# submarine0418/underwater_image_enhancement

Measured on AMD Instinct MI355X. Metric: megapixels/sec enhanced, higher is better.
Workload: dtype f32/f64

## Files before the change

underwater_image_enhancement_amd/csrc/api.hip:

```cpp
#include <cstdarg>
#include <cstdio>
#include <cstring>
#include <type_traits>

#include "common.h"

#include <cstdlib>

namespace uwie {

static thread_local char g_err[512] = "";
static thread_local uwie_ctx *g_ctx = nullptr;
static const Tuning g_default_tuning{};

const Tuning &tune() { return g_ctx ? g_ctx->tune : g_default_tuning; }
uwie_ctx *current_ctx() { return g_ctx; }

void set_error(const char *fmt, ...)
{
    va_list ap;
    va_start(ap, fmt);
    vsnprintf(g_err, sizeof g_err, fmt, ap);
    va_end(ap);
}
// ... 198 lines not shown
        const EntryFuse ef{P.qpart, tune().entry_fuse == 2 ? nullptr : P.gray, P.guess, p->gray_shift};
        UWIE_TRY(launch_cast_classify(ctx, d_in, s, P.kind, nullptr, P.scratch, st, then_airlight && quad_from_cast(p, P) ? &ef : nullptr));
        *kind = P.kind;
    }
    return UWIE_OK;
}

int six_airlight(uwie_ctx *ctx, const uint8_t *d_in, const int32_t *kind, Shape s, const uwie_params *p, const Pipe &P,
                 hipStream_t st, bool after_cast = false)
{
    const bool fused = after_cast && quad_from_cast(p, P);
    return launch_airlight(ctx, d_in, kind, P.gray, s, p->min_size, P.A, nullptr, P.scratch, st,
                           fused && tune().entry_fuse != 2 ? 0 : p->gray_shift, fused ? P.qpart : nullptr);
}

int six_dehaze_tail(uwie_ctx *ctx, const uint8_t *d_in, const int32_t *kind, Shape s, const uwie_params *p, const Pipe &P,
                    uint8_t *d_out_u8, float *d_out_f32, hipStream_t st)
{
    const float eps = 1e-6f;
    const int k = p->strategy;
    int t_is_f32 = 0;
    UWIE_TRY(stage_guided(P, s, p, FuseT0Args{d_in, kind, P.A, (float)p->omega, 1e-6f, 1}, st, &t_is_f32));
    SelectPlan plan;
    const double q[4] = {p->L_low, p->L_high, p->wb_percentile, 100 - p->wb_percentile};
    const RestoreSrc src{d_in, kind, P.A, P.t, t_is_f32};
    bool recompute = false;
    if (tune().select_generic) {
        UWIE_TRY(select_begin<float>(s, q, k == 3 ? 4 : 2, P.scratch, st, &plan));
        UWIE_TRY(launch_restore_planar_hist(d_in, kind, P.A, P.t, s, P.F, plan.ghist, st, false, nullptr, t_is_f32));
        UWIE_TRY(select_run(plan, P.F, 1, s, true, st));
    } else {
        recompute = k != 3 && !tune().restore_store;
        const bool predict = k != 3 || tune().lin_predict3;
        UWIE_TRY(select_lin_begin<float>(s, q, k == 3 ? 4 : 2, P.scratch, st, &plan, predict ? &src : nullptr));
        const bool big = (size_t)s.B * s.npx() >= ((size_t)1 << 24) || tune().rank_sweep >= 2;
        if (recompute && plan.predicted && !t_is_f32 && tune().rank_sweep && big && s.npx() >= 4) {
            UWIE_TRY(launch_restore_rank(src, s, plan, st));
            UWIE_TRY(select_rank_run(plan, s, st, src));
        } else {
            UWIE_TRY(launch_restore_planar_hist(d_in, kind, P.A, P.t, s, recompute ? nullptr : P.F, plan.ghist, st, true,
                                                &plan, t_is_f32));
            UWIE_TRY(select_lin_run(plan, P.F, s, st, recompute ? &src : nullptr));
        }
    }
    if (k == 3) {
        UWIE_TRY(select_lerp_chain(plan, s, eps, P.pct, st));
        return launch_tail_plain(P.F, P.pct, 4, eps, 1, s, 0, 1.0, d_out_u8, d_out_f32, st);
    }
    UWIE_TRY(select_lerp(plan, s, P.pct, st));
    return launch_tail_clahe(ctx, P.F, P.pct, 2, eps, 0, s, p->clip_limit, p->tiles_x, p->tiles_y, k == 1 ? 1 : 0,
                             p->gamma, d_out_u8, d_out_f32, P.scratch, st, recompute ? &src : nullptr);
}

int run_six(uwie_ctx *ctx, const uint8_t *d_in, Shape s, const uwie_params *p, const Pipe &P, uint8_t *d_out_u8,
            float *d_out_f32, hipStream_t st)
{
    const int32_t *kind = nullptr;
    const bool dz = p->strategy >= 1 && p->strategy <= 3;
    UWIE_TRY(six_cast(ctx, d_in, s, p, P, &kind, st, dz));
    if (dz) {
        UWIE_TRY(six_airlight(ctx, d_in, kind, s, p, P, st, true));
        return six_dehaze_tail(ctx, d_in, kind, s, p, P, d_out_u8, d_out_f32, st);
    }
    return launch_code_strategy(ctx, d_in, kind, s, p, d_out_u8, d_out_f32, P.scratch, st);
}

int run_dict_dehaze(uwie_ctx *ctx, const uint8_t *d_in, Shape s, const uwie_params *p, const Pipe &P, uint8_t *d_out_u8,
                    float *d_out_f32, hipStream_t st, double *d_out_f64 = nullptr, bool have_airlight = false)
{
// ... 1759 lines not shown
```

underwater_image_enhancement_amd/csrc/common.h:

```cpp
#pragma once
#include <hip/hip_runtime.h>
#include <stddef.h>
#include <stdint.h>

#include "../../include/uwie.h"

namespace uwie {

void set_error(const char *fmt, ...);
#define UWIE_HIP_CHECK(expr)                                                            \
    do {                                                                                \
        hipError_t _e = (expr);                                                         \
        if (_e != hipSuccess) {                                                         \
            ::uwie::set_error("%s failed: %s (%s:%d)", #expr, hipGetErrorString(_e), __FILE__, __LINE__); \
            return UWIE_E_HIP;                                                          \
        }                                                                               \
    } while (0)
#define UWIE_LAUNCH_CHECK() UWIE_HIP_CHECK(hipGetLastError())
#define UWIE_REQUIRE(cond, msg)                 \
    do {                                        \
        if (!(cond)) {                          \
            ::uwie::set_error("%s", msg);       \
            return UWIE_E_INVALID;              \
        }                                       \
// ... 52 lines not shown
#define UWIE_LAUNCH(kernel, ...) UWIE_LAUNCH_AS(#kernel, kernel, __VA_ARGS__)

}

namespace uwie {
struct Tuning {
    int gf_split = 1;
    int gf_bands = 0;
    int select_generic = 0;
    int restore_store = 0;
    int lin_predict3 = 0;
    int lin_cap = 0;
    int lin_no_predict = 0;
    int q_hist = 1;
    int lin_predict_shift = 0;
    int streams = 1;
    int canny_prepass = 1;
    int gf_fuse = 2;
    int rank_sweep = 1;
    int canny_fault_inject = 0;
    int entry_fuse = 1;
};
const Tuning &tune();
uwie_ctx *current_ctx();
}

struct uwie_ctx {
    int device;
    uwie::Tuning tune;
    bool attr_q_tail = false;
    bool attr_cast_resolve = false;
    int attr_gf_fast = 0;
    int attr_gf_split8 = 0;
    int cus = 0;
    uwie::LabTables *d_lab;
    uwie::CastTables *d_cast;
    uwie::Profiler *prof;
    uint32_t *d_status = nullptr;
    hipStream_t aux[4];
    hipEvent_t fork, join[4];
    bool aux_ready;
    bool last_enhance_f64 = false;
};

namespace uwie {

struct Carver {
    char *base;
    size_t off;
    explicit Carver(void *b) : base(static_cast<char *>(b)), off(0) {}
    template <typename T>
    T *take(size_t count)
    {
        off = (off + 255) & ~size_t(255);
        T *p = base ? reinterpret_cast<T *>(base + off) : nullptr;
        off += count * sizeof(T);
        return p;
    }
    size_t total() const { return (off + 255) & ~size_t(255); }
};

static inline int cdiv(long long a, long long b) { return (int)((a + b - 1) / b); }
static inline int grid_for(size_t n, size_t cap = 8192)
{
    size_t g = (n + 255) / 256;
    if (g > cap) g = cap;
// ... 131 lines not shown
struct FuseT0Args {
    const uint8_t *rgb;
    const int32_t *kind;
    const float *A;
    float omega, norm_eps;
    int pre_clip;
};
int launch_guided_plan(const GuidedPlan &g, Shape s, const uint8_t *d_gray, const void *d_t0, double *d_t, void *ws, hipStream_t st,
                       const FuseT0Args *frame = nullptr);
int guided_fast_th(Shape s, int k);
int launch_guided_fast(const uint8_t *d_gray, const float *d_t0, Shape s, int k, int TH, double eps, double *d_t, hipStream_t st);

constexpr int kMaxPct = 4;
size_t select_ws_bytes(Shape s);
template <typename V>
int launch_percentiles(const V *d_vals, int planar, Shape s, const double *q_percent, int nq, V *d_out, void *ws, hipStream_t st);
int launch_widen_f32(const float *d_in, double *d_out, size_t n, hipStream_t st);

constexpr int kSelGroupStride = 2 * kMaxPct * 2048;
constexpr int kSelOsStride = 2 * kMaxPct;
struct LinState;
struct SelectPlan {
    void *state;
    uint32_t *ghist;
    void *os;
    double t[kMaxPct];
    int nq;
    bool is64;
    LinState *lin;
    void *lists;
    uint32_t *flags;
    uint32_t cap;
    bool predicted;
    uint32_t ranks[2 * kMaxPct];
    template <typename V>
    V *lists_as() const { return static_cast<V *>(lists); }
};
constexpr int kLinBins = 2050;
__host__ __device__ inline uint32_t lin_digit(float x)
{
    if (!(x > 0.0f)) return 0;
    if (x >= 1.0f) return kLinBins - 1;
    const uint32_t d = (uint32_t)(x * 2048.0f);
    return 1 + (d > 2047u ? 2047u : d);
}
__host__ __device__ inline uint32_t lin_digit(double x)
{
    if (!(x > 0.0)) return 0;
    if (x >= 1.0) return kLinBins - 1;
    const uint32_t d = (uint32_t)(x * 2048.0);
    return 1 + (d > 2047u ? 2047u : d);
}
constexpr int kLinLists = 2 * kMaxPct;
constexpr uint32_t kLinNoWin = 0x80000000u;
struct LinState {
    uint32_t rr[2 * kMaxPct];
    uint32_t qbin[2 * kMaxPct];
    uint32_t gid[2 * kMaxPct];
    uint32_t gbin[2 * kMaxPct];
    uint32_t gcount[kLinLists];
    uint32_t ngroups;
    uint32_t wlo[kMaxPct], wspan[kMaxPct];
    uint32_t below[kMaxPct];
};
constexpr int kRankCapMul = 4;
constexpr uint32_t kLinAnyBin = 0xfffffffeu;
struct RestoreSrc;
template <typename V>
int select_lin_begin(Shape s, const double *q_percent, int nq, void *ws, hipStream_t st, SelectPlan *plan,
                     const RestoreSrc *predict = nullptr);
template <typename V>
int select_lin_run(const SelectPlan &plan, const V *d_planar, Shape s, hipStream_t st, const RestoreSrc *src = nullptr);
template <typename V>
int select_begin(Shape s, const double *q_percent, int nq, void *ws, hipStream_t st, SelectPlan *plan);
template <typename V>
int select_run(const SelectPlan &plan, const V *d_vals, int planar, Shape s, bool pass1_done, hipStream_t st);
template <typename V>
int select_lerp(const SelectPlan &plan, Shape s, V *d_out, hipStream_t st);
int select_lerp_chain(const SelectPlan &plan, Shape s, float eps, float *d_pct4, hipStream_t st);
int select_begin_stretch_ranks(Shape s, const float *d_params, int stride, void *ws, hipStream_t st, SelectPlan *plan);
int select_begin_gated_ranks(Shape s, const float *d_params, int stride, uint32_t *d_status, void *ws, hipStream_t st,
                             SelectPlan *plan);
int launch_diff_enhance(const float *d_img, int planar, Shape s, const float *d_params, int flags, const float *d_os,
                        float *d_out, hipStream_t st, float *d_saved = nullptr);
size_t diff_u8_ws_bytes(Shape s);
int launch_diff_enhance_u8(const uint8_t *d_in, Shape s, const float *d_params, int flags, uint8_t *d_out_u8, float *d_out_f32,
                           float *d_saved, void *ws, hipStream_t st);
size_t diff_gated_u8_ws_bytes(int B);
int launch_diff_gated_u8(const uint8_t *d_in, Shape s, const float *d_params, uint32_t *d_status, uint8_t *d_out_u8,
                         float *d_out_f32, float *d_saved, void *ws, hipStream_t st);
int launch_diff_gated(const float *d_img, int planar, Shape s, const float *d_params, const float *d_os, float *d_out,
                      hipStream_t st, float *d_saved = nullptr);
size_t diff_enhance_bwd_ws_bytes(Shape s);
int launch_module_bwd(int map, const float *d_img, int planar, Shape s, const float *d_params, int flags, const float *d_saved,
                      const float *d_ref, const float *d_grad_out, const float *d_grad_loss, float *d_grad_img,
                      float *d_grad_params, void *ws, hipStream_t st);
size_t refloss_ws_bytes(Shape s);
int launch_refloss(int map, const float *d_img, int planar, Shape s, const float *d_params, int flags, const float *d_os,
                   const float *d_ref, float *d_out, float *d_saved, float *d_loss, void *ws, hipStream_t st);
int launch_refloss_bwd(int map, const float *d_img, int planar, Shape s, const float *d_params, int flags, const float *d_saved,
                       const float *d_ref, const float *d_grad_out, const float *d_grad_loss, float *d_grad_img,
                       float *d_grad_params, void *ws, hipStream_t st);
struct VggNet {
// ... 115 lines not shown
```

underwater_image_enhancement_amd/csrc/k_fused.hip:

```cpp
#include <cstdlib>

#include "common.h"
#include "devutil.h"
#include "restore.h"

namespace uwie {

namespace {

typedef uint32_t __attribute__((aligned(1))) u32_unaligned;
typedef uint4 __attribute__((aligned(1))) u128_unaligned;

__device__ __forceinline__ float clip01(float v) { return __builtin_amdgcn_fmed3f(v, 0.0f, 1.0f); }
typedef float f32x2 __attribute__((ext_vector_type(2)));
#ifndef UWIE_CLAHE_PREFETCH
#define UWIE_CLAHE_PREFETCH 0
#endif
#ifndef UWIE_STRETCH_WAVES
#define UWIE_STRETCH_WAVES 5
#endif
__device__ __forceinline__ uint8_t sat_u8(int v) { return (uint8_t)min(max(v, 0), 255); }
#define UWIE_DESCALE(x, n) (((x) + (1 << ((n)-1))) >> (n))

template <bool LIN, bool COLLECT, int NW = 2, typename V = float>
// ... 273 lines not shown
    const uint32_t n = scj;
    const int c = j / kRankNW, w = j % kRankNW;
    uint32_t base = 0;
    if (X.lane == 0) base = atomicAdd(X.gcount0 + (size_t)c * X.gstride + w, n);
    base = (uint32_t)__builtin_amdgcn_readfirstlane((int)base);
    float *L = X.lists0 + ((size_t)c * (kLinLists / kRankCapMul) + w) * X.cap;
    wave_lds_sync();
    for (uint32_t i = X.lane; i < n; i += 64)
        if (base + i < X.cap) L[base + i] = X.mystg[j][i];
    wave_lds_sync();
    scj = 0;
}

__device__ __forceinline__ void rank_exact_batch(const RankWave &X, uint32_t first, uint32_t m, bool counted, uint32_t (&sc)[kRankNS])
{
    wave_lds_sync();
    int jj = -1;
    float x = 0.0f;
    if ((uint32_t)X.lane < m) {
        const uint32_t e = X.myq[first + X.lane];
        const int p = (int)(e >> 2), c = (int)(e & 3u);
        const double tv = X.t[p];
        const uint32_t u = X.img[(size_t)p * 3 + c];
        const float df = X.ftab[c * 256 + (int)u], ac = c == 0 ? X.a0 : c == 1 ? X.a1 : X.a2;
        const double n = (double)df;
        double q;
        if (RestoreImgT<1>::recip_ok(tv)) {
            const double y = RestoreImgT<1>::recip(tv), q0 = n * y;
            q = fma(fma(-tv, q0, n), y, q0);
        } else {
            q = n / tv;
        }
        x = clip01((float)(q + (double)ac));
        const uint32_t d = lin_digit(x);
        const float v32 = fmaf(df, __builtin_amdgcn_rcpf((float)tv), ac);
#pragma unroll
        for (int w = 0; w < kRankNW; ++w) {
            const int j = c * kRankNW + w;
            const uint32_t wlo = X.s_wlo[j];
            if (wlo == kLinNoWin) continue;
            if (counted && !(v32 >= X.s_lo[j] && v32 <= X.s_hi[j])) continue;
            if (d < wlo) atomicAdd(&X.s_below[j], 1u);
            else if (d - wlo <= X.s_wspan[j]) jj = j;
        }
    }
#pragma unroll
    for (int j = 0; j < kRankNS; ++j) {
        const uint64_t mk = __ballot(jj == j);
        if (mk) {
            const uint32_t pos = sc[j] + (uint32_t)__popcll(mk & ((1ull << X.lane) - 1));
            if (jj == j) X.mystg[j][pos] = x;
            sc[j] += (uint32_t)__popcll(mk);
            if (sc[j] >= 64u) rank_flush_stage(X, j, sc[j]);
        }
    }
}

__global__ void __launch_bounds__(256) k_restore_rank(RestoreSrc S, int npx, LinState *__restrict__ lin, float *__restrict__ lists,
                                                      uint32_t cap)
{
    constexpr int NW = kRankNW, NS = kRankNS, QW = kRankQW, SW = kRankSW;
    __shared__ uint32_t wq[4][QW];
    __shared__ float wstg[4][NS][SW];
    __shared__ float ftab[768];
    __shared__ uint32_t s_wlo[NS], s_wspan[NS];
    __shared__ float s_lo[NS], s_hi[NS];
    __shared__ uint32_t s_below[NS];
    const int b = blockIdx.y, tid = threadIdx.x, lane = tid & 63, wv = tid >> 6;
    if (tid < NS) {
        s_below[tid] = 0;
        const LinState &L = lin[3 * b + tid / NW];
        const uint32_t lo = L.wlo[tid % NW], span = L.wspan[tid % NW];
        s_wlo[tid] = lo;
        s_wspan[tid] = span;
        s_lo[tid] = lo == kLinNoWin ? __builtin_inff() : (float)(lo - 1) * (1.0f / 2048.0f) - kRankMargin;
        s_hi[tid] = lo == kLinNoWin ? -__builtin_inff() : (float)(lo + span) * (1.0f / 2048.0f) + kRankMargin;
    }
    RestoreImgT<1> R;
    R.init(S, b, (size_t)npx, ftab);
    __syncthreads();
    float elo[NS], ehi[NS];
#pragma unroll
    for (int j = 0; j < NS; ++j) {
        elo[j] = s_lo[j];
        ehi[j] = s_hi[j];
    }
    const float a0 = R.a[0], a1 = R.a[1], a2 = R.a[2];
    const uint8_t *img = S.in + (size_t)b * npx * 3;
    const double *tpl = S.t + (size_t)b * npx;
    uint32_t *myq = wq[wv];
    uint32_t cnt[NS] = {0, 0, 0, 0, 0, 0};
    uint32_t seen = 0;
    uint32_t qn = 0;
    uint32_t sc[NS] = {0, 0, 0, 0, 0, 0};

    const RankWave X{img, tpl, ftab, a0, a1, a2, s_wlo, s_wspan, s_lo, s_hi, s_below, myq, wstg[wv],
                     &lin[3 * b].gcount[0], (uint32_t)(sizeof(LinState) / sizeof(uint32_t)),
                     lists + (size_t)(3 * b) * (kLinLists / kRankCapMul) * cap, cap, lane};

    const int step = gridDim.x * 1024, iters = (npx + step - 1) / step;
    typedef uint32_t __attribute__((aligned(1))) u32_a1;
#define UWIE_RANK_LOAD4(p_, w_, tv_)                                                                                   \
    do {                                                                                                                \
        const u32_a1 *q_ = reinterpret_cast<const u32_a1 *>(img + (size_t)(p_) * 3);                                    \
        (w_)[0] = q_[0]; (w_)[1] = q_[1]; (w_)[2] = q_[2];                                                              \
        const double2_a8 ta_ = *reinterpret_cast<const double2_a8 *>(tpl + (p_)),                                       \
                         tb_ = *reinterpret_cast<const double2_a8 *>(tpl + (p_) + 2);                                   \
        (tv_)[0] = ta_.x; (tv_)[1] = ta_.y; (tv_)[2] = tb_.x; (tv_)[3] = tb_.y;                                         \
    } while (0)
// ... 890 lines not shown
}

}

void clahe_plan_info(Shape s, double clip, int tx, int ty, bool recomputed, uwie_clahe_plan_info *out)
{
    const ClaheLaunch L = plan_clahe(s, clip, tx, ty, recomputed);
    const ClaheGeom &g = L.g;
    out->tile_w = g.tw;
    out->tile_h = g.th;
    out->padded = L.padded;
    out->clip_limit = g.clip;
    out->wide_lut = L.wide;
    out->nchunk = L.nchunk;
    out->cells_walk = out->cells_flat = 0;
    int rows = 0;
    for (int cyi = 0; cyi <= ty; ++cyi)
        rows += std::max(cyi * g.th - g.th / 2, 0) < std::min((cyi + 1) * g.th - g.th / 2, g.H);
    for (int cxi = 0; cxi <= tx; ++cxi) {
        const int cx0 = std::max(cxi * g.tw - g.tw / 2, 0), cx1 = std::min((cxi + 1) * g.tw - g.tw / 2, g.W);
        if (cx0 >= cx1) continue;
        (clahe_apply_walks((cx1 - cx0 + 3) / 4) ? out->cells_walk : out->cells_flat) += rows;
    }
}

int launch_restore_planar_hist(const uint8_t *d_in, const int32_t *d_kind, const float *d_A, const double *d_t, Shape s,
                               float *d_planar, uint32_t *d_ghist, hipStream_t st, bool linear, const SelectPlan *plan, int t32)
{
    return launch_planar_hist<float>(RestoreSrc{d_in, d_kind, d_A, d_t, t32}, s, d_planar, d_ghist, st, linear, plan);
}

int launch_restore_rank(const RestoreSrc &src, Shape s, const SelectPlan &plan, hipStream_t st)
{
    UWIE_REQUIRE(!src.t32 && plan.nq <= 2 && plan.predicted && s.npx() >= 4, "restore_rank: float64 transmission, two predicted percentiles");
    UWIE_LAUNCH(k_restore_rank, dim3(producer_blocks(5120, s), s.B), dim3(256), 0, st, src, (int)s.npx(), plan.lin, plan.lists_as<float>(),
                (uint32_t)kRankCapMul * plan.cap);
    UWIE_LAUNCH_CHECK();
    return UWIE_OK;
}

int launch_recover64_planar_hist(const uint8_t *d_in, const float *d_A, const double *d_t, Shape s, double *d_planar,
                                 uint32_t *d_ghist, hipStream_t st, bool linear, const SelectPlan *plan)
{
    return launch_planar_hist<double>(RestoreSrc{d_in, nullptr, d_A, d_t}, s, d_planar, d_ghist, st, linear, plan);
}

int launch_tail_plain64(const double *d_planar, const double *d_pct, Shape s, int apply_gamma, double gamma,
                        uint8_t *d_out_u8, float *d_out_f32, hipStream_t st, const RestoreSrc *src, double *d_out_f64)
{
    const dim3 grid(grid_for(s.npx(), 4096), s.B);
    if (src)
        UWIE_LAUNCH(k_stretch64_out<true>, grid, dim3(256), 0, st, d_planar, *src, d_pct, (int)s.npx(), apply_gamma, 1.0 / gamma,
                    d_out_u8, d_out_f32, d_out_f64);
    else
        UWIE_LAUNCH(k_stretch64_out<false>, grid, dim3(256), 0, st, d_planar, RestoreSrc{}, d_pct, (int)s.npx(), apply_gamma,
                    1.0 / gamma, d_out_u8, d_out_f32, d_out_f64);
    UWIE_LAUNCH_CHECK();
    return UWIE_OK;
}

size_t tail_ws_bytes(Shape s, int tx, int ty)
{
    Carver c(nullptr);
    c.take<uint8_t>((size_t)s.B * tx * ty * 256);
    c.take<uint8_t>((size_t)s.B * s.npx() * 3);
    return c.total();
}
// ... 73 lines not shown
```

underwater_image_enhancement_amd/csrc/k_select.hip:

```cpp
#include <cmath>
#include <cstdlib>

#include "common.h"
#include "devutil.h"
#include "restore.h"

namespace uwie {

namespace {

constexpr int kMaxRanks = 2 * kMaxPct;
constexpr int kBins = 2048;

template <typename V>
struct Traits;
template <>
struct Traits<float> {
    using K = uint32_t;
    static constexpr int NPASS = 3;
    __host__ __device__ static int shift(int p) { return p == 0 ? 21 : p == 1 ? 10 : 0; }
    __host__ __device__ static int bits(int p) { return p == 2 ? 10 : 11; }
    __device__ static K key(float v) { return f32_key(v); }
    __device__ static float value(K k) { return __uint_as_float(k ^ ((k >> 31) ? 0x80000000u : 0xffffffffu)); }
};
// ... 345 lines not shown
    out[bc * 4 + 2] = np_lerp<float>(m[0], m[1], fr.t[2]);
    out[bc * 4 + 3] = np_lerp<float>(m[2], m[3], fr.t[3]);
}

template <typename V>
void percentile_indices(long long n, double q_percent, uint32_t *prev, uint32_t *next, double *t)
{
    const V q = (V)q_percent / (V)100;
    const V nm1 = (V)(n - 1);
    const V vi = nm1 * q;
    const V p = std::floor(vi);
    if (vi >= nm1) {
        *prev = *next = (uint32_t)(n - 1);
        *t = 0.0;
        return;
    }
    *prev = (uint32_t)p;
    *next = *prev + 1;
    *t = (double)(vi - p);
}

uint32_t lin_cap(Shape s)
{
    const uint32_t dflt = (uint32_t)std::max<size_t>(65536, s.npx() / 64);
    const long v = tune().lin_cap;
    return v > 0 && v < (long)dflt ? (uint32_t)v : dflt;
}

void carve_select(Carver &c, Shape s, bool lin, SelectPlan *plan)
{
    const size_t nbc = (size_t)s.B * 3;
    plan->state = c.take<SelState<uint64_t>>(nbc);
    plan->ghist = c.take<uint32_t>(nbc * kMaxRanks * kBins);
    plan->os = c.take<double>(nbc * kMaxRanks);
    if (!lin) return;
    plan->lin = c.take<LinState>(nbc);
    plan->flags = c.take<uint32_t>(nbc);
    plan->cap = lin_cap(s);
    plan->lists = c.take<double>(nbc * kLinLists * plan->cap);
}

int zero_ghist(const SelectPlan &plan, Shape s, hipStream_t st)
{
    UWIE_HIP_CHECK(hipMemsetAsync(plan.ghist, 0, sizeof(uint32_t) * (size_t)s.B * 3 * kMaxRanks * kBins, st));
    return UWIE_OK;
}

RankList rank_list(const SelectPlan &plan)
{
    RankList ranks;
    ranks.n = 2 * plan.nq;
    for (int j = 0; j < ranks.n; ++j) ranks.r[j] = plan.ranks[j];
    return ranks;
}

template <typename V>
int plan_percentiles(Shape s, const double *q_percent, int nq, void *ws, bool lin, SelectPlan *plan)
{
    UWIE_REQUIRE(nq >= 1 && nq <= kMaxPct, "percentiles: 1..4 percentiles per call");
    const long long n = (long long)s.npx();
    UWIE_REQUIRE(n >= 1 && n < (1ll << 31), "percentiles: plane size out of range");
    Carver c(ws);
    carve_select(c, s, lin, plan);
    plan->nq = nq;
    plan->is64 = sizeof(V) == 8;
    for (int j = 0; j < nq; ++j)
        percentile_indices<V>(n, q_percent[j], &plan->ranks[2 * j], &plan->ranks[2 * j + 1], &plan->t[j]);
    return UWIE_OK;
}

__global__ void k_sel_init_stretch_ranks(SelState<uint32_t> *st, int nbc, const float *__restrict__ params, int stride,
                                         int n)
{
    const int i = blockIdx.x * blockDim.x + threadIdx.x;
    if (i >= nbc) return;
    const float *pr = params + (size_t)(i / 3) * stride;
    RankList ranks;
// ... 16 lines not shown
    int k[2];
    const bool ok0 = gated_rank(pr[0], n, &k[0]), ok1 = gated_rank(pr[1], n, &k[1]);
    const bool ok = ok0 && ok1;
    RankList ranks;
    ranks.n = 2;
    ranks.r[0] = ok ? (uint32_t)k[0] : 0u;
    ranks.r[1] = ok ? (uint32_t)k[1] : 0u;
    if (!ok && status) atomicOr(status, (uint32_t)UWIE_STATUS_DIFF_RANK);
    st[i] = sel_state<uint32_t>(ranks);
}

template <class Init>
int begin_ranks(Shape s, const char *range_msg, void *ws, hipStream_t st, SelectPlan *plan, Init &&init)
{
    const long long n = (long long)s.npx();
    UWIE_REQUIRE(n >= 1 && n < (1ll << 31), range_msg);
    Carver c(ws);
    carve_select(c, s, false, plan);
    plan->nq = 1;
    plan->is64 = false;
    plan->t[0] = 0.0;
    init((SelState<uint32_t> *)plan->state, s.B * 3, (int)n);
    UWIE_LAUNCH_CHECK();
    return zero_ghist(*plan, s, st);
}

}

namespace {

constexpr uint32_t kLinDone = 0xffffffffu;
constexpr int kLinSampleOff = 4096;

template <typename V>
__global__ void __launch_bounds__(256) k_lin_sample(RestoreSrc S, int npx, int stride, int ngs, uint32_t *__restrict__ ghist)
{
    __shared__ uint32_t h[3][kLinBins];
    const int b = blockIdx.y, tid = threadIdx.x;
    for (int i = tid; i < 3 * kLinBins; i += 256) (&h[0][0])[i] = 0;
    __syncthreads();
    RestoreImg R;
    RestoreImg32 R32;
    if (S.t32) R32.init(S, b, (size_t)npx);
    else R.init(S, b, (size_t)npx);
    for (int i = blockIdx.x * 256 + tid; i < ngs; i += gridDim.x * 256) {
        V r[3][4];
        if constexpr (sizeof(V) == 8) R.four64((i * stride + stride / 2) * 4, 4, r);
        else if (S.t32) R32.four((i * stride + stride / 2) * 4, 4, r);
        else R.four((i * stride + stride / 2) * 4, 4, r);
#pragma unroll
        for (int c = 0; c < 3; ++c)
#pragma unroll
            for (int j = 0; j < 4; ++j) atomicAdd(&h[c][lin_digit(r[c][j])], 1u);
    }
    __syncthreads();
    for (int i = tid; i < 3 * kLinBins; i += 256) {
        const uint32_t c = (&h[0][0])[i];
        if (c) atomicAdd(&ghist[(size_t)(b * 3 + i / kLinBins) * kSelGroupStride + kLinSampleOff + (i % kLinBins)], c);
    }
}

__global__ void __launch_bounds__(256) k_lin_predict(LinState *__restrict__ st, uint32_t *__restrict__ ghist,
                                                     RankList ranks, uint32_t n, uint32_t ns, int shift)
{
    __shared__ uint32_t h[kLinBins], wsum[4], found[2], wl[kMaxPct], wh[kMaxPct];
    const int bc = blockIdx.x, tid = threadIdx.x;
    if (tid < kMaxPct) { wl[tid] = kLinNoWin; wh[tid] = 0; }
    if (ns > 0) {
        uint32_t *gh = ghist + (size_t)bc * kSelGroupStride + kLinSampleOff;
        for (int i = tid; i < kLinBins; i += 256) {
            h[i] = gh[i];
            gh[i] = 0;
        }
        __syncthreads();
        for (int j = 0; j < ranks.n / 2 && j < kMaxPct; ++j) {
            const double p = (double)ranks.r[2 * j] / (double)n, sd = sqrt((double)ns * p * (1.0 - p));
            const double c0 = (double)ranks.r[2 * j] * ns / n, c1 = (double)ranks.r[2 * j + 1] * ns / n, delta = 4.0 * sd + 2.0;
            const uint32_t rlo = (uint32_t)fmax(c0 - delta, 0.0), rhi = (uint32_t)fmin(c1 + delta, (double)ns - 1.0);
            uint32_t dlo, dhi, rr;
            block_find_digit(h, kLinBins, rlo, wsum, found, dlo, rr);
            block_find_digit(h, kLinBins, rhi, wsum, found, dhi, rr);
            if (tid == 0) {
                wl[j] = (uint32_t)min(max((int)dlo + shift, 1), kLinBins - 2);
                wh[j] = (uint32_t)min(max((int)dhi + shift, (int)wl[j]), kLinBins - 2);
            }
        }
    }
    __syncthreads();
    if (tid == 0) {
        LinState s;
        for (int q = 0; q < kMaxRanks; ++q) { s.rr[q] = 0; s.qbin[q] = 0; s.gid[q] = kLinDone; s.gbin[q] = kLinDone; }
        for (int g = 0; g < kLinLists; ++g) s.gcount[g] = 0;
        s.ngroups = 0;
        for (bool again = true; again;) {
            again = false;
            for (int i = 0; i < kMaxPct; ++i)
                for (int j = i + 1; j < kMaxPct; ++j)
                    if (wl[i] != kLinNoWin && wl[j] != kLinNoWin && wl[j] <= wh[i] + 1 && wl[i] <= wh[j] + 1) {
                        wl[i] = min(wl[i], wl[j]);
                        wh[i] = max(wh[i], wh[j]);
                        wl[j] = kLinNoWin;
                        again = true;
                    }
        }
        for (int w = 0; w < kMaxPct; ++w) {
            s.wlo[w] = wl[w];
            s.wspan[w] = wl[w] == kLinNoWin ? 0 : wh[w] - wl[w];
            s.below[w] = 0;
        }
        st[bc] = s;
    }
}

template <typename V>
__global__ void __launch_bounds__(256) k_lin_scan(LinState *__restrict__ st, uint32_t *__restrict__ ghist, RankList ranks,
                                                  V *__restrict__ os, uint32_t *__restrict__ flags, uint32_t cap,
                                                  SelState<typename Traits<V>::K> *__restrict__ sel)
// ... 21 lines not shown
            s.rr[q] = qrr[q];
            s.qbin[q] = qbin[q];
            if (qbin[q] == 0 || qbin[q] == kLinBins - 1) {
                os[bc * kMaxRanks + q] = qbin[q] == 0 ? (V)0 : (V)1;
                continue;
            }
            int w = -1;
            for (int i = kMaxPct - 1; i >= 0; --i)
                if (qbin[q] - s.wlo[i] <= s.wspan[i]) w = i;
            if (w >= 0 && s.gcount[w] > cap) w = -1;
            if (w >= 0) s.gid[q] = (uint32_t)w;
            else covered = false;
        }
        uint32_t ng = 0;
        if (!covered) {
            for (int g = 0; g < kLinLists; ++g) s.gcount[g] = 0;
            for (int q = 0; q < ranks.n; ++q) {
                s.gid[q] = kLinDone;
                if (qbin[q] == 0 || qbin[q] == kLinBins - 1) continue;
                uint32_t g = 0;
                for (; g < ng; ++g)
                    if (s.gbin[g] == qbin[q]) break;
                if (g == ng) s.gbin[ng++] = qbin[q];
                s.gid[q] = g;
            }
        }
        s.ngroups = ng;
        st[bc] = s;
        flags[bc] = 0;
    }
}

__global__ void k_rank_scan(LinState *__restrict__ st, RankList ranks, float *__restrict__ os, uint32_t *__restrict__ flags,
                            uint32_t cap, int nbc, SelState<uint32_t> *__restrict__ sel)
{
    const int bc = blockIdx.x * blockDim.x + threadIdx.x;
    if (bc >= nbc) return;
    sel[bc] = sel_state<uint32_t>(ranks);
    LinState s = st[bc];
    bool miss = false;
    for (int q = 0; q < kMaxRanks; ++q) { s.rr[q] = 0; s.qbin[q] = 0; s.gid[q] = kLinDone; s.gbin[q] = kLinDone; }
    for (int q = 0; q < ranks.n; ++q) {
        const uint32_t r = ranks.r[q];
        bool done = false;
        for (int w = 0; w < kMaxPct && !done; ++w) {
            if (s.wlo[w] == kLinNoWin) continue;
            const uint32_t below = s.below[w], cnt = s.gcount[w];
            if (r >= below && r - below < cnt) {
                if (cnt <= cap) {
                    s.gid[q] = (uint32_t)w;
                    s.rr[q] = r - below;
                    s.qbin[q] = kLinAnyBin;
                } else {
                    miss = true;
                }
                done = true;
            } else if (r < below && s.wlo[w] == 1u) {
                os[bc * kMaxRanks + q] = 0.0f;
                done = true;
            } else if (r >= below && s.wlo[w] + s.wspan[w] == (uint32_t)kLinBins - 2u) {
                os[bc * kMaxRanks + q] = 1.0f;
                done = true;
            }
        }
        miss = miss || !done;
    }
    s.ngroups = 0;
    st[bc] = s;
    flags[bc] = miss ? 1u : 0u;
}

template <typename V>
__global__ void __launch_bounds__(256) k_lin_collect(const V *__restrict__ vals, int n, LinState *__restrict__ st,
                                                     V *__restrict__ lists, uint32_t cap)
{
    constexpr int kStage = sizeof(V) == 8 ? 256 : 512;
    __shared__ V stg[kMaxRanks][kStage];
    __shared__ uint32_t scount[kMaxRanks], sbase[kMaxRanks];
    const int bc = blockIdx.y, tid = threadIdx.x;
    LinState *s = st + bc;
    const int ng = (int)s->ngroups;
    if (ng == 0) return;
    uint32_t gd[kMaxRanks];
#pragma unroll
    for (int g = 0; g < kMaxRanks; ++g) gd[g] = g < ng ? s->gbin[g] - 1 : kLinDone;
    if (tid < kMaxRanks) scount[tid] = 0;
    __syncthreads();
    V *L = lists + (size_t)bc * kLinLists * cap;
    const V *v = vals + (size_t)bc * n;
    const int per = (((n + 3) / 4 + gridDim.x - 1) / gridDim.x) * 4;
    const int lo = min(n, blockIdx.x * per), hi = min(n, lo + per);
    auto take = [&](V x, bool live) {
        const uint32_t d = (live && x > (V)0) ? (uint32_t)(x * (V)2048) : 0xfffffffeu;
// ... 121 lines not shown
            for (uint32_t i = tid; i < c; i += 256)
                if (base + i < cap) L[base + i] = stg[j][i];
        }
        __syncthreads();
        if (tid < 3 * NG) scount[tid] = 0;
        __syncthreads();
    };
    constexpr int U = 2;
    for (int base = lo; base < hi; base += U * 1024) {
#pragma unroll
        for (int u = 0; u < U; ++u) {
            const int p = base + u * 1024 + tid * 4, m = min(4, hi - p);
            if (m > 0) {
                V r[3][4];
                if constexpr (sizeof(V) == 8) R.four64(p, m, r);
                else if (S.t32) R32.four(p, m, r);
                else R.four(p, m, r);
#pragma unroll
                for (int i = 0; i < 4; ++i) {
                    take(0, r[0][i], i < m);
                    take(1, r[1][i], i < m);
                    take(2, r[2][i], i < m);
                }
            }
        }
        flush(false);
    }
    flush(true);
}

template <typename V>
__global__ void __launch_bounds__(1024) k_lin_finish(const LinState *__restrict__ st, const V *__restrict__ lists,
                                                     uint32_t cap, V *__restrict__ os, uint32_t *__restrict__ flags, int pair,
                                                     int nlists)
{
    using K = typename Traits<V>::K;
    constexpr int kBuf = 49152 / (int)sizeof(V);
    __shared__ uint32_t h[2048], wsum[16], found[2], s_nloc;
    __shared__ unsigned long long s_kmin, s_kmax;
    __shared__ V s_buf[kBuf];
    const int bc = blockIdx.x, tid = threadIdx.x, lane = tid & 63;
    const LinState *s = st + bc;
    int q = blockIdx.y;
    if (pair) {
        const int half = (int)gridDim.y / 2;
        if (q < half) {
            q = 2 * q;
        } else {
            q = 2 * (q - half) + 1;
            if (s->gid[q] != kLinDone && s->gid[q] == s->gid[q - 1] && s->qbin[q] == s->qbin[q - 1] && s->rr[q] - s->rr[q - 1] <= 1u)
                return;
        }
    }
    const bool with_next = pair && !(q & 1);
    const uint32_t g = s->gid[q];
    if (g == kLinDone) return;
    const uint32_t cnt = s->gcount[g];
    if (cnt > cap) {
        if (tid == 0) flags[bc] = 1;
        return;
    }
    const V *L = lists + ((size_t)bc * nlists + g) * cap;
    uint32_t r = s->rr[q];
    const uint32_t tb = s->qbin[q];
    bool sub = false;
    float sub_lo = 0.0f, sub_scale = 0.0f;
    uint32_t sub_d = 0;
    auto subbin = [&](V x) -> uint32_t {
        const float f = ((float)x - sub_lo) * sub_scale;
        return (uint32_t)fminf(fmaxf(f, 0.0f), 2047.0f);
    };
    if (tb == kLinAnyBin && cnt > (uint32_t)kBuf) {
        sub = true;
        sub_lo = (float)(s->wlo[g] - 1u) * (1.0f / 2048.0f);
        sub_scale = 2048.0f * 2048.0f / (float)(s->wspan[g] + 1u);
        for (int i = tid; i < 2048; i += 1024) h[i] = 0;
        __syncthreads();
        constexpr int kFly = sizeof(V) == 4 ? 16 : 8;
        for (uint32_t base = 0; base < cnt; base += kFly * 1024) {
            V x[kFly];
#pragma unroll
            for (int u = 0; u < kFly; ++u) {
                const uint32_t i = min(base + u * 1024 + tid, cnt - 1);
                x[u] = L[i];
            }
#pragma unroll
            for (int u = 0; u < kFly; ++u)
                if (base + u * 1024 + tid < cnt) atomicAdd(&h[subbin(x[u])], 1u);
        }
        __syncthreads();
        uint32_t d, rr;
        block_find_digit(h, 2048, r, wsum, found, d, rr);
        sub_d = d;
        r = rr;
    }
    const uint32_t r_mine = r;
    auto is_mine = [&](V x, uint32_t i) -> bool {
        if (tb != kLinAnyBin) return lin_digit(x) == tb;
        return i < cnt && (!sub || subbin(x) == sub_d);
    };
    if (tid == 0) {
        s_nloc = 0;
        s_kmin = ~0ull;
        s_kmax = 0ull;
    }
    __syncthreads();
    {
        unsigned long long kmin = ~0ull, kmax = 0ull;
// ... 129 lines not shown
            const unsigned long long a = shfl_u64(kgt, lane ^ o);
            kgt = a < kgt ? a : kgt;
        }
        if (lane == 0) atomicMin(&s_kmin, kgt);
        __syncthreads();
    }
    if (tid == 0) os[bc * kMaxRanks + q1] = Traits<V>::value((K)(s_nloc > r_mine + 1u ? prefix : s_kmin));
}

template <typename V>
struct LinRows;
template <>
struct LinRows<float> {
    static constexpr const char *sample = "k_lin_sample<float>", *scan = "k_lin_scan<float>", *collect = "k_lin_collect<float>",
                                *collect_src = "(k_lin_collect_src<float, 4>)", *finish = "k_lin_finish<float>";
};
template <>
struct LinRows<double> {
    static constexpr const char *sample = "k_lin_sample<double>", *scan = "k_lin_scan<double>", *collect = "k_lin_collect<double>",
                                *collect_src = "k_lin_collect_src64", *finish = "k_lin_finish<double>";
};

}

size_t select_ws_bytes(Shape s)
{
    Carver c(nullptr);
    SelectPlan plan;
    carve_select(c, s, true, &plan);
    return c.total();
}

template <typename V>
int select_lin_begin(Shape s, const double *q_percent, int nq, void *ws, hipStream_t st, SelectPlan *plan, const RestoreSrc *predict)
{
    constexpr bool f64 = sizeof(V) == 8;
    int rc = plan_percentiles<V>(s, q_percent, nq, ws, true, plan);
    if (rc == UWIE_OK) rc = zero_ghist(*plan, s, st);
    if (rc != UWIE_OK) return rc;
    const int n = (int)s.npx(), nbc = s.B * 3;
    const int ngroups = n / 4;
    plan->predicted = predict && !tune().lin_no_predict && (!f64 || (nq <= 2 && ngroups > 0));
    uint32_t ns = 0;
    if (plan->predicted && ngroups > 0) {
        int stride = std::max(1, ngroups / 32768);
        if (stride > 1) stride |= 1;
        const int ngs = ngroups / stride;
        ns = 4u * (uint32_t)ngs;
        UWIE_LAUNCH_AS(LinRows<V>::sample, k_lin_sample<V>, dim3(std::max(1, std::min(8, cdiv(ngs, 512))), s.B), dim3(256), 0, st,
                       *predict, n, stride, ngs, plan->ghist);
        UWIE_LAUNCH_CHECK();
    }
    UWIE_LAUNCH(k_lin_predict, dim3(nbc), dim3(256), 0, st, plan->lin, plan->ghist, rank_list(*plan), (uint32_t)n, ns,
                tune().lin_predict_shift);
    UWIE_LAUNCH_CHECK();
    return UWIE_OK;
}

template <typename V>
int select_lin_run(const SelectPlan &plan, const V *d_planar, Shape s, hipStream_t st, const RestoreSrc *src)
{
    using Rows = LinRows<V>;
    const int n = (int)s.npx(), nbc = s.B * 3;
    const RankList ranks = rank_list(plan);
    UWIE_REQUIRE(!src || ranks.n <= 4, "select_lin_run: the recomputing sweep handles at most two percentiles");
    V *lists = plan.lists_as<V>(), *os = (V *)plan.os;
    UWIE_LAUNCH_AS(Rows::scan, k_lin_scan<V>, dim3(nbc), dim3(256), 0, st, plan.lin, plan.ghist, ranks, os, plan.flags, plan.cap,
                   (SelState<typename Traits<V>::K> *)plan.state);
    UWIE_LAUNCH_CHECK();
    int blocks = (int)(((long long)n + 131071) / 131072);
    if (blocks * nbc < 1024) blocks = cdiv(1024, nbc);
    blocks = blocks < 1 ? 1 : blocks > 256 ? 256 : blocks;
    if (plan.predicted) blocks = std::max(1, std::min(2 * blocks, cdiv(24576, nbc)));
    if (src) {
        const int per_image = std::min(3 * blocks, std::max(1, cdiv(n, 2048)));
        UWIE_LAUNCH_AS(Rows::collect_src, (k_lin_collect_src<V, 4>), dim3(per_image, s.B), dim3(256), 0, st, *src, n, plan.lin, lists,
                       plan.cap);
    } else {
        UWIE_LAUNCH_AS(Rows::collect, k_lin_collect<V>, dim3(blocks, nbc), dim3(256), 0, st, d_planar, n, plan.lin, lists, plan.cap);
    }
    UWIE_LAUNCH_CHECK();
    UWIE_LAUNCH_AS(Rows::finish, k_lin_finish<V>, dim3(nbc, ranks.n), dim3(1024), 0, st, plan.lin, lists, plan.cap, os,
                   plan.flags, 0, kLinLists);
    UWIE_LAUNCH_CHECK();
    if (src) return sel_passes(plan, RestoredVals<V>{*src, n}, n, nbc, pass_blocks(n, nbc, true), false, plan.flags, st);
    const StoredVals<V> vals{d_planar, (size_t)n * 3, (size_t)n, 1};
    return sel_passes(plan, vals, n, nbc, pass_blocks(n, nbc, false), false, plan.flags, st);
}

template int select_lin_begin<float>(Shape, const double *, int, void *, hipStream_t, SelectPlan *, const RestoreSrc *);
template int select_lin_run<float>(const SelectPlan &, const float *, Shape, hipStream_t, const RestoreSrc *);
template int select_lin_begin<double>(Shape, const double *, int, void *, hipStream_t, SelectPlan *, const RestoreSrc *);
template int select_lin_run<double>(const SelectPlan &, const double *, Shape, hipStream_t, const RestoreSrc *);

int select_rank_run(const SelectPlan &plan, Shape s, hipStream_t st, const RestoreSrc &src)
{
    const int n = (int)s.npx(), nbc = s.B * 3;
    const RankList ranks = rank_list(plan);
    UWIE_LAUNCH(k_rank_scan, dim3(cdiv(nbc, 64)), dim3(64), 0, st, plan.lin, ranks, (float *)plan.os, plan.flags, kRankCapMul * plan.cap,
                nbc, (SelState<uint32_t> *)plan.state);
    UWIE_LAUNCH_CHECK();
    UWIE_LAUNCH(k_lin_finish<float>, dim3(nbc, ranks.n), dim3(1024), 0, st, plan.lin, plan.lists_as<float>(),
                kRankCapMul * plan.cap, (float *)plan.os, plan.flags, 1, kLinLists / kRankCapMul);
    UWIE_LAUNCH_CHECK();
    return sel_passes(plan, RestoredVals<float>{src, n}, n, nbc, pass_blocks(n, nbc, true), false, plan.flags, st);
}

int select_begin_stretch_ranks(Shape s, const float *d_params, int stride, void *ws, hipStream_t st, SelectPlan *plan)
{
    return begin_ranks(s, "stretch ranks: plane size out of range", ws, st, plan, [&](SelState<uint32_t> *state, int nbc, int n) {
        UWIE_LAUNCH(k_sel_init_stretch_ranks, dim3(cdiv(nbc, 64)), dim3(64), 0, st, state, nbc, d_params, stride, n);
    });
}

int select_begin_gated_ranks(Shape s, const float *d_params, int stride, uint32_t *d_status, void *ws, hipStream_t st,
                             SelectPlan *plan)
{
    return begin_ranks(s, "gated ranks: plane size out of range", ws, st, plan, [&](SelState<uint32_t> *state, int nbc, int n) {
        UWIE_LAUNCH(k_sel_init_gated_ranks, dim3(cdiv(nbc, 64)), dim3(64), 0, st, state, nbc, d_params, stride, n, d_status);
    });
}

int select_lerp_chain(const SelectPlan &plan, Shape s, float eps, float *d_pct4, hipStream_t st)
{
    UWIE_REQUIRE(plan.nq == 4 && !plan.is64, "chained stretch needs 4 float32 percentiles");
    FracList<float> fr;
    fr.n = 4;
    for (int j = 0; j < 4; ++j) fr.t[j] = (float)plan.t[j];
    const int nbc = s.B * 3;
    UWIE_LAUNCH(k_pct_finish_chain, dim3(cdiv(nbc, 64)), dim3(64), 0, st, (const float *)plan.os, nbc, fr, eps, d_pct4);
    UWIE_LAUNCH_CHECK();
    return UWIE_OK;
}

template <typename V>
int select_begin(Shape s, const double *q_percent, int nq, void *ws, hipStream_t st, SelectPlan *plan)
// ... 68 lines not shown
```

Measured before the change: 60100.

## Use 8x finer sample histogram bins for rank-route percentile window prediction

```diff
diff --git a/underwater_image_enhancement_amd/csrc/api.hip b/underwater_image_enhancement_amd/csrc/api.hip
--- a/underwater_image_enhancement_amd/csrc/api.hip
+++ b/underwater_image_enhancement_amd/csrc/api.hip
@@ -254,9 +254,10 @@
     } else {
         recompute = k != 3 && !tune().restore_store;
         const bool predict = k != 3 || tune().lin_predict3;
-        UWIE_TRY(select_lin_begin<float>(s, q, k == 3 ? 4 : 2, P.scratch, st, &plan, predict ? &src : nullptr));
         const bool big = (size_t)s.B * s.npx() >= ((size_t)1 << 24) || tune().rank_sweep >= 2;
-        if (recompute && plan.predicted && !t_is_f32 && tune().rank_sweep && big && s.npx() >= 4) {
+        const bool rank_route = recompute && !t_is_f32 && tune().rank_sweep && big && s.npx() >= 4;
+        UWIE_TRY(select_lin_begin<float>(s, q, k == 3 ? 4 : 2, P.scratch, st, &plan, predict ? &src : nullptr, rank_route));
+        if (plan.rank) {
             UWIE_TRY(launch_restore_rank(src, s, plan, st));
             UWIE_TRY(select_rank_run(plan, s, st, src));
         } else {
diff --git a/underwater_image_enhancement_amd/csrc/common.h b/underwater_image_enhancement_amd/csrc/common.h
--- a/underwater_image_enhancement_amd/csrc/common.h
+++ b/underwater_image_enhancement_amd/csrc/common.h
@@ -108,6 +108,7 @@
     bool attr_cast_resolve = false;
     int attr_gf_fast = 0;
     int attr_gf_split8 = 0;
+    bool attr_lin_fine = false;
     int cus = 0;
     uwie::LabTables *d_lab;
     uwie::CastTables *d_cast;
@@ -305,6 +306,7 @@
     uint32_t *flags;
     uint32_t cap;
     bool predicted;
+    bool rank;
     uint32_t ranks[2 * kMaxPct];
     template <typename V>
     V *lists_as() const { return static_cast<V *>(lists); }
@@ -323,6 +325,15 @@
     if (x >= 1.0) return kLinBins - 1;
     const uint32_t d = (uint32_t)(x * 2048.0);
     return 1 + (d > 2047u ? 2047u : d);
+}
+constexpr int kLinFine = 8;
+constexpr int kLinFineBins = 2 + 2048 * kLinFine;
+__host__ __device__ inline uint32_t lin_digit_fine(float x)
+{
+    if (!(x > 0.0f)) return 0;
+    if (x >= 1.0f) return kLinFineBins - 1;
+    const uint32_t d = (uint32_t)(x * 16384.0f);
+    return 1 + (d > 16383u ? 16383u : d);
 }
 constexpr int kLinLists = 2 * kMaxPct;
 constexpr uint32_t kLinNoWin = 0x80000000u;
@@ -341,7 +352,7 @@
 struct RestoreSrc;
 template <typename V>
 int select_lin_begin(Shape s, const double *q_percent, int nq, void *ws, hipStream_t st, SelectPlan *plan,
-                     const RestoreSrc *predict = nullptr);
+                     const RestoreSrc *predict = nullptr, bool rank_route = false);
 template <typename V>
 int select_lin_run(const SelectPlan &plan, const V *d_planar, Shape s, hipStream_t st, const RestoreSrc *src = nullptr);
 template <typename V>
diff --git a/underwater_image_enhancement_amd/csrc/k_fused.hip b/underwater_image_enhancement_amd/csrc/k_fused.hip
--- a/underwater_image_enhancement_amd/csrc/k_fused.hip
+++ b/underwater_image_enhancement_amd/csrc/k_fused.hip
@@ -329,7 +329,7 @@
             q = n / tv;
         }
         x = clip01((float)(q + (double)ac));
-        const uint32_t d = lin_digit(x);
+        const uint32_t d = lin_digit_fine(x);
         const float v32 = fmaf(df, __builtin_amdgcn_rcpf((float)tv), ac);
 #pragma unroll
         for (int w = 0; w < kRankNW; ++w) {
@@ -370,8 +370,9 @@
         const uint32_t lo = L.wlo[tid % NW], span = L.wspan[tid % NW];
         s_wlo[tid] = lo;
         s_wspan[tid] = span;
-        s_lo[tid] = lo == kLinNoWin ? __builtin_inff() : (float)(lo - 1) * (1.0f / 2048.0f) - kRankMargin;
-        s_hi[tid] = lo == kLinNoWin ? -__builtin_inff() : (float)(lo + span) * (1.0f / 2048.0f) + kRankMargin;
+        constexpr float kUnit = 1.0f / (float)(kLinFineBins - 2);
+        s_lo[tid] = lo == kLinNoWin ? __builtin_inff() : (float)(lo - 1) * kUnit - kRankMargin;
+        s_hi[tid] = lo == kLinNoWin ? -__builtin_inff() : (float)(lo + span) * kUnit + kRankMargin;
     }
     RestoreImgT<1> R;
     R.init(S, b, (size_t)npx, ftab);
@@ -1328,7 +1329,8 @@
 
 int launch_restore_rank(const RestoreSrc &src, Shape s, const SelectPlan &plan, hipStream_t st)
 {
-    UWIE_REQUIRE(!src.t32 && plan.nq <= 2 && plan.predicted && s.npx() >= 4, "restore_rank: float64 transmission, two predicted percentiles");
+    UWIE_REQUIRE(!src.t32 && plan.nq <= 2 && plan.predicted && plan.rank && s.npx() >= 4,
+                 "restore_rank: float64 transmission, two percentiles predicted in fine bins");
     UWIE_LAUNCH(k_restore_rank, dim3(producer_blocks(5120, s), s.B), dim3(256), 0, st, src, (int)s.npx(), plan.lin, plan.lists_as<float>(),
                 (uint32_t)kRankCapMul * plan.cap);
     UWIE_LAUNCH_CHECK();
diff --git a/underwater_image_enhancement_amd/csrc/k_select.hip b/underwater_image_enhancement_amd/csrc/k_select.hip
--- a/underwater_image_enhancement_amd/csrc/k_select.hip
+++ b/underwater_image_enhancement_amd/csrc/k_select.hip
@@ -401,6 +401,7 @@
     const size_t nbc = (size_t)s.B * 3;
     plan->state = c.take<SelState<uint64_t>>(nbc);
     plan->ghist = c.take<uint32_t>(nbc * kMaxRanks * kBins);
+    plan->rank = false;
     plan->os = c.take<double>(nbc * kMaxRanks);
     if (!lin) return;
     plan->lin = c.take<LinState>(nbc);
@@ -411,7 +412,9 @@
 
 int zero_ghist(const SelectPlan &plan, Shape s, hipStream_t st)
 {
-    UWIE_HIP_CHECK(hipMemsetAsync(plan.ghist, 0, sizeof(uint32_t) * (size_t)s.B * 3 * kMaxRanks * kBins, st));
+    size_t bytes = sizeof(uint32_t) * (size_t)s.B * 3 * kMaxRanks * kBins;
+    if (plan.rank) bytes = (size_t)((char *)plan.os - (char *)plan.ghist) + sizeof(double) * (size_t)s.B * 3 * kMaxRanks;
+    UWIE_HIP_CHECK(hipMemsetAsync(plan.ghist, 0, bytes, st));
     return UWIE_OK;
 }
 
@@ -494,18 +497,23 @@
 constexpr uint32_t kLinDone = 0xffffffffu;
 constexpr int kLinSampleOff = 4096;
 
-template <typename V>
-__global__ void __launch_bounds__(256) k_lin_sample(RestoreSrc S, int npx, int stride, int ngs, uint32_t *__restrict__ ghist)
-{
-    __shared__ uint32_t h[3][kLinBins];
+constexpr int kFineWords = kLinFineBins / 2 + 1;
+constexpr int kFineEndStride = kMaxRanks * sizeof(double) / sizeof(uint32_t);
+constexpr int kFineSampleThreads = 512;
+template <typename V, bool FINE>
+__global__ void __launch_bounds__(FINE ? kFineSampleThreads : 256) k_lin_sample(RestoreSrc S, int npx, int stride, int ngs,
+                                                                               uint32_t *__restrict__ ghist, uint32_t *__restrict__ ends)
+{
+    constexpr int NT = FINE ? kFineSampleThreads : 256, NH = FINE ? 3 * kFineWords : 3 * kLinBins;
+    extern __shared__ uint32_t h[];
     const int b = blockIdx.y, tid = threadIdx.x;
-    for (int i = tid; i < 3 * kLinBins; i += 256) (&h[0][0])[i] = 0;
+    for (int i = tid; i < NH; i += NT) h[i] = 0;
     __syncthreads();
     RestoreImg R;
     RestoreImg32 R32;
     if (S.t32) R32.init(S, b, (size_t)npx);
     else R.init(S, b, (size_t)npx);
-    for (int i = blockIdx.x * 256 + tid; i < ngs; i += gridDim.x * 256) {
+    for (int i = blockIdx.x * NT + tid; i < ngs; i += gridDim.x * NT) {
         V r[3][4];
         if constexpr (sizeof(V) == 8) R.four64((i * stride + stride / 2) * 4, 4, r);
         else if (S.t32) R32.four((i * stride + stride / 2) * 4, 4, r);
@@ -513,38 +521,98 @@
 #pragma unroll
         for (int c = 0; c < 3; ++c)
 #pragma unroll
-            for (int j = 0; j < 4; ++j) atomicAdd(&h[c][lin_digit(r[c][j])], 1u);
-    }
-    __syncthreads();
-    for (int i = tid; i < 3 * kLinBins; i += 256) {
-        const uint32_t c = (&h[0][0])[i];
-        if (c) atomicAdd(&ghist[(size_t)(b * 3 + i / kLinBins) * kSelGroupStride + kLinSampleOff + (i % kLinBins)], c);
-    }
+            for (int j = 0; j < 4; ++j) {
+                if constexpr (FINE) {
+                    const uint32_t slot = lin_digit_fine(r[c][j]) + 1u;
+                    atomicAdd(&h[c * kFineWords + (slot >> 1)], 1u << (16 * (slot & 1u)));
+                } else {
+                    atomicAdd(&h[c * kLinBins + lin_digit(r[c][j])], 1u);
+                }
+            }
+    }
+    __syncthreads();
+    for (int i = tid; i < NH; i += NT) {
+        const uint32_t c = h[i];
+        if constexpr (FINE) {
+            const int bc = b * 3 + i / kFineWords, w = i % kFineWords;
+            if (!c) continue;
+            if (w == 0) {
+                atomicAdd(&ends[bc * kFineEndStride], c >> 16);
+            } else if (w == kFineWords - 1) {
+                atomicAdd(&ends[bc * kFineEndStride + 1], c & 0xffffu);
+            } else {
+                uint32_t *g = ghist + (size_t)bc * kSelGroupStride + 2 * (w - 1);
+                atomicAdd(reinterpret_cast<unsigned long long *>(g), (unsigned long long)(c & 0xffffu) | ((unsigned long long)(c >> 16) << 32));
+            }
+        } else {
+            if (c) atomicAdd(&ghist[(size_t)(b * 3 + i / kLinBins) * kSelGroupStride + kLinSampleOff + (i % kLinBins)], c);
+        }
+    }
+}
+int lin_sample_grid(int ngs, bool fine)
+{
+    const int nt = fine ? kFineSampleThreads : 256;
+    int blocks = std::max(1, std::min(2048 / nt, cdiv(ngs, 2 * nt)));
+    if (fine) blocks = std::max(blocks, cdiv(ngs, (65535 / (4 * nt)) * nt));
+    return blocks;
+}
+long long lin_sample_block_values(int ngs, int blocks, int nt)
+{
+    const long long round = (long long)blocks * nt;
+    return 4 * ((ngs / round) * nt + std::min<long long>(nt, ngs % round));
 }
 
 __global__ void __launch_bounds__(256) k_lin_predict(LinState *__restrict__ st, uint32_t *__restrict__ ghist,
-                                                     RankList ranks, uint32_t n, uint32_t ns, int shift)
-{
-    __shared__ uint32_t h[kLinBins], wsum[4], found[2], wl[kMaxPct], wh[kMaxPct];
+                                                     const uint32_t *__restrict__ ends, int nbins, RankList ranks, uint32_t n,
+                                                     uint32_t ns, int shift)
+{
+    extern __shared__ uint32_t hs[];
+    __shared__ uint32_t wsum[4], found[2], wl[kMaxPct], wh[kMaxPct];
     const int bc = blockIdx.x, tid = threadIdx.x;
+    const int R = (nbins - 2) / (kLinBins - 2);
+    uint32_t *h = hs, *hf = hs + kLinBins;
     if (tid < kMaxPct) { wl[tid] = kLinNoWin; wh[tid] = 0; }
     if (ns > 0) {
-        uint32_t *gh = ghist + (size_t)bc * kSelGroupStride + kLinSampleOff;
-        for (int i = tid; i < kLinBins; i += 256) {
-            h[i] = gh[i];
-            gh[i] = 0;
-        }
-        __syncthreads();
+        if (R == 1) {
+            uint32_t *gh = ghist + (size_t)bc * kSelGroupStride + kLinSampleOff;
+            for (int i = tid; i < kLinBins; i += 256) {
+                h[i] = gh[i];
+                gh[i] = 0;
+            }
+        } else {
+            uint32_t *gh = ghist + (size_t)bc * kSelGroupStride;
+            for (int i = tid; i < nbins - 2; i += 256) {
+                hf[1 + i] = gh[i];
+                gh[i] = 0;
+            }
+            if (tid < 2) hf[tid * (nbins - 1)] = ends[bc * kFineEndStride + tid];
+            __syncthreads();
+            for (int i = tid; i < kLinBins; i += 256) {
+                uint32_t c = i == 0 ? hf[0] : i == kLinBins - 1 ? hf[nbins - 1] : 0u;
+                if (i > 0 && i < kLinBins - 1)
+                    for (int k = 0; k < R; ++k) c += hf[1 + (i - 1) * R + k];
+                h[i] = c;
+            }
+        }
+        __syncthreads();
+        auto find = [&](uint32_t r) -> uint32_t {
+            uint32_t d, rr;
+            block_find_digit(h, kLinBins, r, wsum, found, d, rr);
+            if (R == 1 || d == 0) return d;
+            if (d == (uint32_t)kLinBins - 1) return (uint32_t)nbins - 1;
+            uint32_t f = 1 + (d - 1) * R;
+            if (tid == 0)
+                for (int k = 0; k < R - 1 && rr >= hf[f]; ++k) rr -= hf[f++];
+            return f;
+        };
         for (int j = 0; j < ranks.n / 2 && j < kMaxPct; ++j) {
             const double p = (double)ranks.r[2 * j] / (double)n, sd = sqrt((double)ns * p * (1.0 - p));
             const double c0 = (double)ranks.r[2 * j] * ns / n, c1 = (double)ranks.r[2 * j + 1] * ns / n, delta = 4.0 * sd + 2.0;
             const uint32_t rlo = (uint32_t)fmax(c0 - delta, 0.0), rhi = (uint32_t)fmin(c1 + delta, (double)ns - 1.0);
-            uint32_t dlo, dhi, rr;
-            block_find_digit(h, kLinBins, rlo, wsum, found, dlo, rr);
-            block_find_digit(h, kLinBins, rhi, wsum, found, dhi, rr);
+            const uint32_t dlo = find(rlo), dhi = find(rhi);
             if (tid == 0) {
-                wl[j] = (uint32_t)min(max((int)dlo + shift, 1), kLinBins - 2);
-                wh[j] = (uint32_t)min(max((int)dhi + shift, (int)wl[j]), kLinBins - 2);
+                wl[j] = (uint32_t)min(max((int)dlo + shift * R, 1), nbins - 2);
+                wh[j] = (uint32_t)min(max((int)dhi + shift * R, (int)wl[j]), nbins - 2);
             }
         }
     }
@@ -632,7 +700,7 @@
 }
 
 __global__ void k_rank_scan(LinState *__restrict__ st, RankList ranks, float *__restrict__ os, uint32_t *__restrict__ flags,
-                            uint32_t cap, int nbc, SelState<uint32_t> *__restrict__ sel)
+                            uint32_t cap, int nbc, SelState<uint32_t> *__restrict__ sel, uint32_t nbins)
 {
     const int bc = blockIdx.x * blockDim.x + threadIdx.x;
     if (bc >= nbc) return;
@@ -658,7 +726,7 @@
             } else if (r < below && s.wlo[w] == 1u) {
                 os[bc * kMaxRanks + q] = 0.0f;
                 done = true;
-            } else if (r >= below && s.wlo[w] + s.wspan[w] == (uint32_t)kLinBins - 2u) {
+            } else if (r >= below && s.wlo[w] + s.wspan[w] == nbins - 2u) {
                 os[bc * kMaxRanks + q] = 1.0f;
                 done = true;
             }
@@ -846,7 +914,7 @@
 template <typename V>
 __global__ void __launch_bounds__(1024) k_lin_finish(const LinState *__restrict__ st, const V *__restrict__ lists,
                                                      uint32_t cap, V *__restrict__ os, uint32_t *__restrict__ flags, int pair,
-                                                     int nlists)
+                                                     int nlists, float wbins)
 {
     using K = typename Traits<V>::K;
     constexpr int kBuf = 49152 / (int)sizeof(V);
@@ -886,8 +954,8 @@
     };
     if (tb == kLinAnyBin && cnt > (uint32_t)kBuf) {
         sub = true;
-        sub_lo = (float)(s->wlo[g] - 1u) * (1.0f / 2048.0f);
-        sub_scale = 2048.0f * 2048.0f / (float)(s->wspan[g] + 1u);
+        sub_lo = (float)(s->wlo[g] - 1u) * (1.0f / wbins);
+        sub_scale = 2048.0f * wbins / (float)(s->wspan[g] + 1u);
         for (int i = tid; i < 2048; i += 1024) h[i] = 0;
         __syncthreads();
         constexpr int kFly = sizeof(V) == 4 ? 16 : 8;
@@ -1083,27 +1151,53 @@
 }
 
 template <typename V>
-int select_lin_begin(Shape s, const double *q_percent, int nq, void *ws, hipStream_t st, SelectPlan *plan, const RestoreSrc *predict)
+int select_lin_begin(Shape s, const double *q_percent, int nq, void *ws, hipStream_t st, SelectPlan *plan, const RestoreSrc *predict,
+                     bool rank_route)
 {
     constexpr bool f64 = sizeof(V) == 8;
     int rc = plan_percentiles<V>(s, q_percent, nq, ws, true, plan);
-    if (rc == UWIE_OK) rc = zero_ghist(*plan, s, st);
     if (rc != UWIE_OK) return rc;
     const int n = (int)s.npx(), nbc = s.B * 3;
     const int ngroups = n / 4;
     plan->predicted = predict && !tune().lin_no_predict && (!f64 || (nq <= 2 && ngroups > 0));
+    plan->rank = !f64 && rank_route && plan->predicted && ngroups > 0;
+    const bool fine = plan->rank;
+    rc = zero_ghist(*plan, s, st);
+    if (rc != UWIE_OK) return rc;
+    constexpr size_t kSampleLds = 3 * kFineWords * sizeof(uint32_t), kPredictLds = (kLinBins + kLinFineBins) * sizeof(uint32_t);
+    if (fine) {
+        uwie_ctx *ctx = current_ctx();
+        if (!ctx || !ctx->attr_lin_fine) {
+            if constexpr (!f64)
+                UWIE_HIP_CHECK(hipFuncSetAttribute(reinterpret_cast<const void *>(&k_lin_sample<float, true>),
+                                                   hipFuncAttributeMaxDynamicSharedMemorySize, (int)kSampleLds));
+            UWIE_HIP_CHECK(hipFuncSetAttribute(reinterpret_cast<const void *>(&k_lin_predict), hipFuncAttributeMaxDynamicSharedMemorySize,
+                                               (int)kPredictLds));
+            if (ctx) ctx->attr_lin_fine = true;
+        }
+    }
     uint32_t ns = 0;
     if (plan->predicted && ngroups > 0) {
         int stride = std::max(1, ngroups / 32768);
         if (stride > 1) stride |= 1;
         const int ngs = ngroups / stride;
         ns = 4u * (uint32_t)ngs;
-        UWIE_LAUNCH_AS(LinRows<V>::sample, k_lin_sample<V>, dim3(std::max(1, std::min(8, cdiv(ngs, 512))), s.B), dim3(256), 0, st,
-                       *predict, n, stride, ngs, plan->ghist);
+        const int blocks = lin_sample_grid(ngs, fine);
+        if (fine) {
+            if constexpr (!f64) {
+                UWIE_REQUIRE(lin_sample_block_values(ngs, blocks, kFineSampleThreads) <= 65535,
+                             "lin sample: a block would file more values of a plane than a 16-bit counter holds");
+                UWIE_LAUNCH_AS(LinRows<V>::sample, (k_lin_sample<float, true>), dim3(blocks, s.B), dim3(kFineSampleThreads), kSampleLds, st,
+                               *predict, n, stride, ngs, plan->ghist, (uint32_t *)plan->os);
+            }
+        } else {
+            UWIE_LAUNCH_AS(LinRows<V>::sample, (k_lin_sample<V, false>), dim3(blocks, s.B), dim3(256), 3 * kLinBins * sizeof(uint32_t), st,
+                           *predict, n, stride, ngs, plan->ghist, (uint32_t *)nullptr);
+        }
         UWIE_LAUNCH_CHECK();
     }
-    UWIE_LAUNCH(k_lin_predict, dim3(nbc), dim3(256), 0, st, plan->lin, plan->ghist, rank_list(*plan), (uint32_t)n, ns,
-                tune().lin_predict_shift);
+    UWIE_LAUNCH(k_lin_predict, dim3(nbc), dim3(256), fine ? kPredictLds : kLinBins * sizeof(uint32_t), st, plan->lin, plan->ghist,
+                (const uint32_t *)plan->os, fine ? kLinFineBins : kLinBins, rank_list(*plan), (uint32_t)n, ns, tune().lin_predict_shift);
     UWIE_LAUNCH_CHECK();
     return UWIE_OK;
 }
@@ -1132,27 +1226,28 @@
     }
     UWIE_LAUNCH_CHECK();
     UWIE_LAUNCH_AS(Rows::finish, k_lin_finish<V>, dim3(nbc, ranks.n), dim3(1024), 0, st, plan.lin, lists, plan.cap, os,
-                   plan.flags, 0, kLinLists);
+                   plan.flags, 0, kLinLists, (float)(kLinBins - 2));
     UWIE_LAUNCH_CHECK();
     if (src) return sel_passes(plan, RestoredVals<V>{*src, n}, n, nbc, pass_blocks(n, nbc, true), false, plan.flags, st);
     const StoredVals<V> vals{d_planar, (size_t)n * 3, (size_t)n, 1};
     return sel_passes(plan, vals, n, nbc, pass_blocks(n, nbc, false), false, plan.flags, st);
 }
 
-template int select_lin_begin<float>(Shape, const double *, int, void *, hipStream_t, SelectPlan *, const RestoreSrc *);
+template int select_lin_begin<float>(Shape, const double *, int, void *, hipStream_t, SelectPlan *, const RestoreSrc *, bool);
 template int select_lin_run<float>(const SelectPlan &, const float *, Shape, hipStream_t, const RestoreSrc *);
-template int select_lin_begin<double>(Shape, const double *, int, void *, hipStream_t, SelectPlan *, const RestoreSrc *);
+template int select_lin_begin<double>(Shape, const double *, int, void *, hipStream_t, SelectPlan *, const RestoreSrc *, bool);
 template int select_lin_run<double>(const SelectPlan &, const double *, Shape, hipStream_t, const RestoreSrc *);
 
 int select_rank_run(const SelectPlan &plan, Shape s, hipStream_t st, const RestoreSrc &src)
 {
     const int n = (int)s.npx(), nbc = s.B * 3;
     const RankList ranks = rank_list(plan);
+    UWIE_REQUIRE(plan.rank, "select_rank_run: the plan's windows are not in fine bins");
     UWIE_LAUNCH(k_rank_scan, dim3(cdiv(nbc, 64)), dim3(64), 0, st, plan.lin, ranks, (float *)plan.os, plan.flags, kRankCapMul * plan.cap,
-                nbc, (SelState<uint32_t> *)plan.state);
+                nbc, (SelState<uint32_t> *)plan.state, (uint32_t)kLinFineBins);
     UWIE_LAUNCH_CHECK();
     UWIE_LAUNCH(k_lin_finish<float>, dim3(nbc, ranks.n), dim3(1024), 0, st, plan.lin, plan.lists_as<float>(),
-                kRankCapMul * plan.cap, (float *)plan.os, plan.flags, 1, kLinLists / kRankCapMul);
+                kRankCapMul * plan.cap, (float *)plan.os, plan.flags, 1, kLinLists / kRankCapMul, (float)(kLinFineBins - 2));
     UWIE_LAUNCH_CHECK();
     return sel_passes(plan, RestoredVals<float>{src, n}, n, nbc, pass_blocks(n, nbc, true), false, plan.flags, st);
 }
```

After: 58980. -1.9%, worse.
